# HKPolyU-UAV/MLMapping

Measured on NVIDIA B200. Metric: rays_integrated_per_sec, higher is better.
Workload: dtype f64

## Files before the change

### mlmapping_b200/csrc/explore_kernels.cuh

```cuda
#pragma once
#include "frame_kernels.cuh"
#include "order_kernels.cuh"

namespace mlm {

__device__ __forceinline__ bool inside_exp_bd(const MapParams &P, double x, double y, double z) {
  return x >= P.bd[0] && x < P.bd[1] && y >= P.bd[2] && y < P.bd[3] && z >= P.bd[4] && z < P.bd[5];
}

__device__ __forceinline__ void miss_tkey_body(const MapParams &P, DeviceBuffers &D, const FrameParams &F) {
  const FrameCounters *fc = D.fc[F.parity];
  const int n = fc->n_miss_list;
  const uint32_t *am = D.act_miss[F.parity];
  for (int j = blockIdx.x * blockDim.x + threadIdx.x; j < n; j += gridDim.x * blockDim.x) {
    const unsigned long long key = ((unsigned long long)am[D.miss_bucket[j]] << 32) | D.miss_t[j];
    atomicMax(&D.lvg_tkey[D.miss_lv[j]], key);
  }
}

__device__ __forceinline__ void nb_of(const MapParams &P, int dir, const int g[3], int sub, int gn[3], int &subn, int dl[3]) {
  int c[3] = {sub % P.n, (sub / P.n) % P.n, sub / (P.n * P.n)};
  gn[0] = g[0];
  gn[1] = g[1];
  gn[2] = g[2];
// ... 49 lines not shown
      if (!pack_glb(gn, hkey)) {
        fc->error = kErrRange;
        continue;
      }
      uint32_t slot = ht_hash(hkey) & P.ht_mask;
      int val = kBlockPending, created = -1;
      bool found = false;
      for (uint32_t probe = 0; probe <= P.ht_mask; probe++) {
        uint64_t k = D.ht_key[slot];
        if (k == kEmptyKey) {
          unsigned long long old = atomicCAS(reinterpret_cast<unsigned long long *>(&D.ht_key[slot]),
                                             (unsigned long long)kEmptyKey, (unsigned long long)hkey);
          if (old == kEmptyKey) {
            int top = atomicSub(D.free_top, 1) - 1;
            if (top < 0) {
              atomicAdd(D.free_top, 1);
              D.ht_val[slot] = kBlockUnusable;
              fc->error = kErrPool;
            } else {
              created = D.free_stack[top];
              D.ht_val[slot] = created;
              atomicAdd(&fc->n_new_blocks, 1);
            }
            val = kBlockPending;
            found = true;
            break;
          }
          k = (uint64_t)old;
        }
        if (k == hkey) {
          val = D.ht_val[slot];
          found = true;
          break;
        }
        slot = (slot + 1) & P.ht_mask;
      }
      if (!found) {
        fc->error = kErrPool;
        continue;
      }
      if (val == kBlockCollapsed || val == kBlockUnusable) continue;
      bool is_u = true;
      if (val >= 0) {
        is_u = D.pool_occ[(size_t)val * P.cell_stride + subn] == 'u';
        if (is_u) {
          const int cn[3] = {c[0] + dl[0], c[1] + dl[1], c[2] + dl[2]};
          const int lx = cn[0] - F.lvg_base[0], ly = cn[1] - F.lvg_base[1], lz = cn[2] - F.lvg_base[2];
          if ((unsigned)lx < (unsigned)P.lvg_dim_xy && (unsigned)ly < (unsigned)P.lvg_dim_xy && (unsigned)lz < (unsigned)P.lvg_dim_z) {
            const int lvn = (lz * P.lvg_dim_xy + ly) * P.lvg_dim_xy + lx;
            if (D.lvg[lvn].y > 0 && D.lvg_tkey[lvn] > my_key) is_u = false;
          }
        }
      }
      if (is_u) {
        const int blk = val >= 0 ? val : created;
        if (blk >= 0) atomicOr(&D.pool_front[(size_t)blk * P.front_words + (subn >> 5)], 1u << (subn & 31));
        else D.miss_choice[j] = (signed char)i;
        break;
      }
    }
  }
}

__device__ __forceinline__ void explore_b_body(const MapParams &P, DeviceBuffers &D, const FrameParams &F) {
  const FrameCounters *fc = D.fc[F.parity];
  const int n = fc->n_miss_list;
  const int dxy = P.lvg_dim_xy;
  for (int j = blockIdx.x * blockDim.x + threadIdx.x; j < n; j += gridDim.x * blockDim.x) {
    const int i = D.miss_choice[j];
    if (i < 0) continue;
    const int lv = D.miss_lv[j];
    int c[3] = {lv % dxy + F.lvg_base[0], (lv / dxy) % dxy + F.lvg_base[1], lv / (dxy * dxy) + F.lvg_base[2]};
    int g[3], l[3];
    for (int a = 0; a < 3; a++) {
      g[a] = floor_div(c[a], P.n);
      l[a] = c[a] - g[a] * P.n;
    }
    int gn[3], subn, dl[3];
    nb_of(P, i, g, (l[2] * P.n + l[1]) * P.n + l[0], gn, subn, dl);
    const int val = ht_find(P, D, gn);
    if (val >= 0) atomicOr(&D.pool_front[(size_t)val * P.front_words + (subn >> 5)], 1u << (subn & 31));
  }
}

__device__ __forceinline__ void release_body(const MapParams &P, DeviceBuffers &D, const FrameParams &F) {
  FrameCounters *fc = D.fc[F.parity];
  const int lane = lane_id();
  const int warp = (blockIdx.x * blockDim.x + threadIdx.x) >> 5, nwarps = (gridDim.x * blockDim.x) >> 5;
  const int n = fc->n_obs;
  for (int o = warp; o < n; o += nwarps) {
    const int ls = D.obs_list[o];
    if (lane == 0) D.obs_flag[ls] = 0;
    int lx = ls % P.lsg_dim_xy, ly = (ls / P.lsg_dim_xy) % P.lsg_dim_xy, lz = ls / (P.lsg_dim_xy * P.lsg_dim_xy);
    int g[3] = {lx + F.lsg_base[0], ly + F.lsg_base[1], lz + F.lsg_base[2]};
    uint32_t slot;
    const int block = ht_find_slot(P, D, g, slot);
    if (block < 0) continue;
    const size_t base = (size_t)block * P.cell_stride;
    bool ok = true;
    for (int w = lane; w < P.front_words; w += 32) ok &= D.pool_front[(size_t)block * P.front_words + w] == 0;
    const char first = D.pool_occ[base];
    if ((base & 3) == 0) {
      const uint32_t first4 = 0x01010101u * (uint32_t)(unsigned char)first;
      const uint32_t *occ4 = reinterpret_cast<const uint32_t *>(D.pool_occ + base);
      const int n4 = P.cells >> 2;
      for (int i = lane; i < n4; i += 32) ok &= occ4[i] == first4;
      for (int i = (n4 << 2) + lane; i < P.cells; i += 32) ok &= D.pool_occ[base + i] == first;
    } else {
      for (int i = lane; i < P.cells; i += 32) ok &= D.pool_occ[base + i] == first;
    }
    if (!__all_sync(0xffffffffu, ok)) continue;
    if (lane == 0) {
      D.col_occ[slot] = first;
      D.col_inf[slot] = D.pool_inf[base];
      D.col_lo[slot] = D.pool_lo[base];
      D.ht_val[slot] = kBlockCollapsed;
      atomicAdd(&fc->n_released, 1);
    }
    __syncwarp();
    for (int i = lane; i < P.cell_stride; i += 32) {
      D.pool_occ[base + i] = 'u';
      D.pool_inf[base + i] = 'u';
      D.pool_lo[base + i] = 0.f;
    }
    for (int w = lane; w < P.front_words; w += 32) D.pool_front[(size_t)block * P.front_words + w] = 0;
    __syncwarp();
    if (lane == 0) {
      __threadfence();
      D.free_stack[atomicAdd(D.free_top, 1)] = block;
    }
  }
}

__global__ void __launch_bounds__(256) k_miss_finalize(MapParams P, DeviceBuffers D, FrameParams F) { miss_finalize_body(P, D, F); }
__global__ void __launch_bounds__(256) k_miss_tkey(MapParams P, DeviceBuffers D, FrameParams F) { miss_tkey_body(P, D, F); }
__global__ void __launch_bounds__(256) k_explore_a(MapParams P, DeviceBuffers D, FrameParams F) { explore_a_body(P, D, F); }
__global__ void __launch_bounds__(256) k_explore_b(MapParams P, DeviceBuffers D, FrameParams F) { explore_b_body(P, D, F); }
__global__ void __launch_bounds__(256) k_release(MapParams P, DeviceBuffers D, FrameParams F) { release_body(P, D, F); }

template <int kMode>
__global__ void __launch_bounds__(kColThreads, 1) k_frame_explore(MapParams P, DeviceBuffers D, FrameParams F) {
  extern __shared__ __align__(16) unsigned char s_raw[];
  const int G = (int)gridDim.x;
  FrameCounters *fc = D.fc[F.parity];
  MLM_FRAME_WALL(0);
  {
    const int n_tiles = (F.n_total + F.tile_pts - 1) / F.tile_pts;
    for (int t = blockIdx.x; t < max(n_tiles, 1); t += G) {
      project_tile<kMode>(P, D, F, t, reinterpret_cast<int *>(s_raw));
      __syncthreads();
    }
  }
  MLM_FRAME_WALL(1);
  grid_barrier(D.grid_bar, G);
  MLM_FRAME_WALL(2);
  column_phase(P, D, F, s_raw);
  MLM_FRAME_WALL(3);
  grid_barrier(D.grid_bar, 2 * G);
  MLM_FRAME_WALL(4);
  if (blockIdx.x == 0 && threadIdx.x == 0) *D.col_queue = 0;
  miss_finalize_body(P, D, F);
  if (__ldcg(&fc->n_hit) > (int)F.bucket_count || __ldcg(&fc->n_miss_list) > (int)F.bucket_count_miss) {
    frame_bail(D, fc, F);
    return;
  }
  fuse_body<1>(P, D, F);
  MLM_FRAME_WALL(5);
  grid_barrier(D.grid_bar, 3 * G);
  miss_tkey_body(P, D, F);
  MLM_FRAME_WALL(6);
  grid_barrier(D.grid_bar, 4 * G);
  explore_a_body(P, D, F);
  MLM_FRAME_WALL(9);
  grid_barrier(D.grid_bar, 5 * G);
  explore_b_body(P, D, F);
  MLM_FRAME_WALL(10);
  fuse_body<2, false>(P, D, F);
  MLM_FRAME_WALL(11);
  grid_barrier(D.grid_bar, 6 * G);
  release_body(P, D, F);
  MLM_FRAME_WALL(12);
  frame_finish(P, D, F, fc, __ldcg(&fc->n_hit));
}

}
```

### mlmapping_b200/csrc/frame_kernels.cuh

```cuda
#pragma once
#include "exact_math.cuh"
#include "types.cuh"

namespace mlm {


__device__ __forceinline__ int cvt_trunc_x86(double x) {
  if (!(x > -2147483649.0 && x < 2147483648.0)) return (int)0x80000000;
  return __double2int_rz(x);
}

__device__ __forceinline__ int lane_id() { return threadIdx.x & 31; }

__device__ __forceinline__ int round_to_int_x86(double v) {
  if (!(v > -2147483000.0 && v < 2147483000.0)) return cvt_trunc_x86(round(v));
  int zi = __double2int_rz(v);
  double frac = v - (double)zi;
  if (frac >= 0.5) zi++;
  else if (frac <= -0.5) zi--;
  return zi;
}

__device__ __forceinline__ int agg_inc(int *ctr) {
  unsigned mask = __activemask();
// ... 547 lines not shown
    __syncwarp();
  }
  __syncthreads();
}

__device__ __forceinline__ void resolve_one(const MapParams &P, const FrameParams &F, DeviceBuffers &D, FrameCounters *fc,
                                            const int ls, const bool rearm_flag) {
  int block = -3;
  int lx = ls % P.lsg_dim_xy, ly = (ls / P.lsg_dim_xy) % P.lsg_dim_xy, lz = ls / (P.lsg_dim_xy * P.lsg_dim_xy);
  int g[3] = {lx + F.lsg_base[0], ly + F.lsg_base[1], lz + F.lsg_base[2]};
  uint64_t key;
  if (!pack_glb(g, key)) {
    fc->error = kErrRange;
  } else {
    uint32_t slot = ht_hash(key) & P.ht_mask;
    bool done = false;
    for (uint32_t probe = 0; probe <= P.ht_mask && !done; probe++) {
      uint64_t k = __ldcg(&D.ht_key[slot]);
      if (k == kEmptyKey) {
        unsigned long long old = atomicCAS(reinterpret_cast<unsigned long long *>(&D.ht_key[slot]),
                                           (unsigned long long)kEmptyKey, (unsigned long long)key);
        if (old == kEmptyKey) {
          int top = atomicSub(D.free_top, 1) - 1;
          if (top < 0) {
            atomicAdd(D.free_top, 1);
            D.ht_val[slot] = -3;
            fc->error = kErrPool;
          } else {
            block = D.free_stack[top];
            D.ht_val[slot] = block;
            atomicAdd(&fc->n_new_blocks, 1);
          }
          done = true;
          break;
        }
        k = (uint64_t)old;
      }
      if (k == key) {
        block = __ldcg(&D.ht_val[slot]);
        if (block == kBlockUnusable) fc->error = kErrPool;
        done = true;
        break;
      }
      slot = (slot + 1) & P.ht_mask;
    }
    if (!done) fc->error = kErrPool;
  }
  D.lsg_block[ls] = block;
  if (rearm_flag) D.lsg_flag[ls] = 0;
}
__device__ __forceinline__ void resolve_subboxes(const MapParams &P, const FrameParams &F, DeviceBuffers &D,
                                                 FrameCounters *fc, int first, int stride) {
  const int n = *reinterpret_cast<volatile int *>(&fc->n_touched_sub);
  for (int i = first; i < n; i += stride) resolve_one(P, F, D, fc, __ldcg(&D.touched_sub[i]), true);
}

__device__ __forceinline__ void touch_subbox(const MapParams &P, const FrameParams &F, DeviceBuffers &D,
                                             FrameCounters *fc, const int g[3]) {
  int ls = lsg_index(P, F, g);
  if (ls < 0) {
    fc->error = kErrInternal;
    return;
  }
  if (__ldcg(&D.lsg_flag[ls]) == 0) {
    if (atomicExch(&D.lsg_flag[ls], 1) == 0) {
      int pos = atomicAdd(&fc->n_touched_sub, 1);
      D.touched_sub[pos] = ls;
      if (F.inline_resolve) resolve_one(P, F, D, fc, ls, false);
    }
  }
}

struct WalkStart {
  double rate;
  int rho, z;
};
__device__ __forceinline__ WalkStart walk_prepare(const MapParams &P, int rho, int z) {
  WalkStart ws;
  ws.rate = (rho < P.nRho && z >= 0 && z < P.nZ) ? __ldg(&P.rate_table[z * P.nRho + rho]) : ray_rate(P, rho, z);
  if (rho >= P.nRho) {
    z = round_to_int_x86((double)z - (double)(rho - P.nRho + 1) * ws.rate);
    rho = P.nRho - 1;
  }
  ws.rho = rho;
  ws.z = z;
  return ws;
}
__device__ __forceinline__ void walk_mark(const MapParams &P, uint32_t *s_miss, double rate, int rho, int z,
                                          uint32_t *stamp_col, uint32_t t) {
  const int lane = lane_id();
  const double zd = (double)z;
  const int w_top = (rho - 1) >> 5;
  double diff = (double)(rho - (w_top << 5) - lane);
  for (int w = w_top; w >= 0; --w, diff += 32.0) {
    const int r = (w << 5) + lane;
    bool valid = r >= 1 && r <= rho - 1;
    const int zc = round_to_int_x86(zd - diff * rate);
    valid = valid && zc >= 0 && zc < P.nZ;
    if (stamp_col && valid) atomicMin(&stamp_col[zc * P.nRho + r], t * (uint32_t)P.nRho + (uint32_t)(rho - 1 - r));
    const int key = valid ? zc : -1;
    const int prev = __shfl_up_sync(0xffffffffu, key, 1);
    const unsigned heads = __ballot_sync(0xffffffffu, lane == 0 || key != prev);
    if (valid && (lane == 0 || key != prev)) {
      const unsigned rest = lane < 31 ? heads >> (lane + 1) : 0u;
      const int len = rest ? __ffs(rest) : 32 - lane;
      const unsigned mask = (len >= 32 ? 0xffffffffu : ((1u << len) - 1u)) << lane;
      uint32_t *wp = &s_miss[zc * P.words_per_row + w];
      if ((*reinterpret_cast<volatile uint32_t *>(wp) & mask) != mask) atomicOr(wp, mask);
    }
  }
}
__device__ __forceinline__ void walk_batch(const MapParams &P, uint32_t *s_miss, bool need, int rho, int z,
                                           uint32_t *stamp_col = nullptr, uint32_t t = 0) {
  WalkStart ws;
  ws.rate = 0.0;
  ws.rho = 0;
  ws.z = 0;
  if (need) ws = walk_prepare(P, rho, z);
  unsigned todo = __ballot_sync(0xffffffffu, need);
  while (todo) {
    const int src = __ffs(todo) - 1;
    todo &= todo - 1;
    const double rate = __shfl_sync(0xffffffffu, ws.rate, src);
    const int r0 = __shfl_sync(0xffffffffu, ws.rho, src);
    const int z0 = __shfl_sync(0xffffffffu, ws.z, src);
    const uint32_t t0 = __shfl_sync(0xffffffffu, t, src);
    walk_mark(P, s_miss, rate, r0, z0, stamp_col, t0);
  }
}

__device__ __forceinline__ void group_bar(int id, int count) { asm volatile("bar.sync %0, %1;" ::"r"(id), "r"(count) : "memory"); }

__device__ __forceinline__ void compact_bits(const uint32_t *bm, int w0, int w1, uint32_t *list, int *counter, int warp,
                                             int nwarps) {
  const int lane = lane_id();
  for (int wi = w0 + warp; wi < w1; wi += nwarps) {
    const uint32_t bits = bm[wi];
    if (!bits) continue;
    int base = 0;
    if (lane == 0) base = atomicAdd(counter, __popc(bits));
    base = __shfl_sync(0xffffffffu, base, 0);
    if ((bits >> lane) & 1u) list[base + __popc(bits & ((1u << lane) - 1))] = ((uint32_t)wi << 5) | (uint32_t)lane;
  }
}

__host__ __device__ inline size_t col_smem_prefix_bytes(int col_words, int nRho, int nCol) {
  return (((size_t)2 * col_words + kCntTotal + kColWarps + (size_t)kOddsRows * nRho + nRho + kMapCap) * 4 + (size_t)nCol * 2 + 15) & ~(size_t)15;
}

#ifdef MLM_PHASE_TIMING
#define MLM_PHASE(i) do { __syncthreads(); if (threadIdx.x == 0) D.debug_cycles[vc * 16 + (i)] = clock64(); } while (0)
#define MLM_PHASE_G(i, leader) do { if (threadIdx.x == (leader)) D.debug_cycles[vc * 16 + (i)] = clock64(); } while (0)
#define MLM_WALL(i) do { if (threadIdx.x == 0) { unsigned long long t_; asm volatile("mov.u64 %0, %%globaltimer;" : "=l"(t_)); D.debug_cycles[vc * 16 + (i)] = (long long)t_; } } while (0)
#else
#define MLM_WALL(i) do { } while (0)
#define MLM_PHASE(i) do { } while (0)
#define MLM_PHASE_G(i, leader) do { } while (0)
#endif

constexpr uint32_t kMissStampPending = 0xffffffffu;
__device__ __forceinline__ void miss_finalize_body(const MapParams &P, DeviceBuffers &D, const FrameParams &F) {
  if (!P.explore || !P.split) return;
  const FrameCounters *fc = D.fc[F.parity];
  const int n = __ldcg(&fc->n_miss_list);
  const int per_z = P.nRho * P.nPhi;
  for (int j = blockIdx.x * blockDim.x + threadIdx.x; j < n; j += gridDim.x * blockDim.x) {
    if (__ldcg(&D.miss_t[j]) != kMissStampPending) continue;
    const int idx = __ldcg(&D.miss_idx[j]);
    const int z = idx / per_z, rem = idx - z * per_z;
    const int phi = rem / P.nRho, r = rem - phi * P.nRho;
    const uint32_t st = __ldcg(&D.miss_stamp[((size_t)phi * P.nZ + z) * P.nRho + r]);
    D.miss_t[j] = st;
    atomicMin(&D.act_miss[F.parity][__ldcg(&D.miss_bucket[j])], st);
  }
}

__device__ __forceinline__ void column_item(const MapParams &P, DeviceBuffers &D, const FrameParams &F, const int item,
                                            unsigned char *s_raw) {
  FrameCounters *fc = D.fc[F.parity];
  uint32_t *act = D.act[F.parity];
  const bool merged = P.split && item >= P.nCol;
  const int phi = merged ? item - P.nCol : (P.split ? item >> 1 : item);
  const int side = (P.split && !merged) ? (item & 1) : -1;
  const int vc = merged ? 2 * phi : item;
  const int vc2 = merged ? vc + 1 : -1;
  const int z_own_lo = side == 1 ? P.n_below + 1 : 0;
  const int z_own_hi = side == 0 ? P.n_below : P.nZ;
  const int z_shared = side >= 0 ? P.n_below : -1;
  const int tid = threadIdx.x;
  const int n_c = D.phi_hist[vc] + (merged ? D.phi_hist[vc2] : 0);
  uint32_t *g_miss = D.miss_bitmap + (size_t)phi * P.col_words;
  MLM_PHASE(15);
  MLM_WALL(13);
  uint32_t *s_miss = reinterpret_cast<uint32_t *>(s_raw);
  uint32_t *s_end = s_miss + P.col_words;
  uint32_t *s_cnt = s_end + P.col_words;
  uint32_t *s_wsum = s_cnt + kCntTotal;
  float *s_odds = reinterpret_cast<float *>(s_wsum + kColWarps);
  int *s_reach = reinterpret_cast<int *>(s_odds + kOddsRows * P.nRho);
  int *s_map = s_reach + P.nRho;
  uint64_t *s_keys = reinterpret_cast<uint64_t *>(s_raw + col_smem_prefix_bytes(P.col_words, P.nRho, P.nCol));
  uint32_t *end_t_col = P.explore ? D.end_t + (size_t)phi * P.nZ * P.nRho : nullptr;
  uint32_t *stamp_col = P.explore ? D.miss_stamp + (size_t)phi * P.nZ * P.nRho : nullptr;
  if (P.explore) {
    const int e_lo = side == 1 ? P.n_below : z_own_lo;
    for (int i = e_lo * P.nRho + tid; i < z_own_hi * P.nRho; i += blockDim.x) end_t_col[i] = 0xffffffffu;
    for (int i = z_own_lo * P.nRho + tid; i < z_own_hi * P.nRho; i += blockDim.x)
      if (!P.split || i < P.n_below * P.nRho || i >= (P.n_below + 1) * P.nRho) stamp_col[i] = 0xffffffffu;
  }
  __shared__ int s_warp[33];
  __shared__ int s_off;
  const int bound_c = D.phi_bound[vc] + (merged ? D.phi_bound[vc2] : 0);
  const bool in_smem = bound_c <= P.sort_cap_smem;
  const bool big = n_c > P.map_cap;
  int off = 0;
  if (big || !in_smem) {
    int part = 0;
    for (int p = tid; p < vc; p += blockDim.x) part += D.phi_hist[p];
    for (int ofs = 16; ofs > 0; ofs >>= 1) part += __shfl_xor_sync(0xffffffffu, part, ofs);
    if (tid == 0) s_off = 0;
    __syncthreads();
    if (lane_id() == 0 && part) atomicAdd(&s_off, part);
    __syncthreads();
    off = s_off;
  }
  {
    const int nb = (F.n_total + F.tile_pts - 1) / F.tile_pts;
    const int per = (nb + (int)blockDim.x - 1) / (int)blockDim.x;
    const int b0 = min(tid * per, nb), b1 = min(b0 + per, nb);
    uint32_t dsave[4], dsave2[4];
    int mine = 0;
#pragma unroll
    for (int q = 0; q < 4; q++) {
      dsave[q] = 0;
      dsave2[q] = 0;
      if (b0 + q < b1) {
        dsave[q] = __ldcg(&D.rec_dir[(size_t)(b0 + q) * P.nCol + vc]);
        mine += (int)(dsave[q] & 0xffffu);
        if (merged) {
          dsave2[q] = __ldcg(&D.rec_dir[(size_t)(b0 + q) * P.nCol + vc2]);
          mine += (int)(dsave2[q] & 0xffffu);
        }
      }
    }
    for (int b = b0 + 4; b < b1; b++) {
      mine += (int)(__ldcg(&D.rec_dir[(size_t)b * P.nCol + vc]) & 0xffffu);
      if (merged) mine += (int)(__ldcg(&D.rec_dir[(size_t)b * P.nCol + vc2]) & 0xffffu);
    }
    int incl = mine;
    const int lane = lane_id(), w = tid >> 5, nw = blockDim.x >> 5;
#pragma unroll
    for (int ofs = 1; ofs < 32; ofs <<= 1) {
      int t = __shfl_up_sync(0xffffffffu, incl, ofs);
      if (lane >= ofs) incl += t;
    }
    if (lane == 31) s_warp[w] = incl;
    __syncthreads();
    if (w == 0) {
      int sv = lane < nw ? s_warp[lane] : 0, si = sv;
#pragma unroll
      for (int ofs = 1; ofs < 32; ofs <<= 1) {
        int t = __shfl_up_sync(0xffffffffu, si, ofs);
        if (lane >= ofs) si += t;
      }
      if (lane < nw) s_warp[lane] = si - sv;
    }
    __syncthreads();
    int dst = s_warp[w] + incl - mine;
    for (int b = b0; b < b1; b++) {
      for (int half = 0; half < (merged ? 2 : 1); half++) {
        const int col = half ? vc2 : vc;
        const uint32_t d = b - b0 < 4 ? (half ? dsave2[b - b0] : dsave[b - b0]) : __ldcg(&D.rec_dir[(size_t)b * P.nCol + col]);
        const int c = (int)(d & 0xffffu);
        const int src = b * F.tile_pts + (int)(d >> 16);
        for (int r = 0; r < c; r++) {
          if (big) D.rec_col[off + dst + r] = D.rec_lin[src + r];
          else s_map[dst + r] = src + r;
        }
        dst += c;
      }
    }
  }
  __syncthreads();
  const RayRecord *recs = big ? D.rec_col + off : D.rec_lin;
#define REC_AT(i) recs[big ? (i) : s_map[i]]
  MLM_PHASE(0);

  __shared__ int s_nk;
  __shared__ int s_nmiss;
  __shared__ int s_nhead;
  __shared__ int s_nlist;
  for (int i = tid; i < 2 * P.col_words; i += blockDim.x) s_miss[i] = 0;
  if (tid == 0) {
    s_nk = 0;
    s_nmiss = 0;
    s_nhead = 0;
  }
  __syncthreads();
  uint64_t *keys = in_smem ? s_keys : D.col_scratch + (size_t)2 * off * P.contrib_per_point;
  uint64_t *keys_alt = in_smem ? s_keys + P.sort_cap_smem : keys + (size_t)n_c * P.contrib_per_point;
  int kbits = 1;
  while ((1 << kbits) < n_c) kbits++;
  const int cell_shift = 12 + kbits;
  const int cell_sentinel = 1 << P.cell_bits;
  __syncthreads();

  MLM_PHASE(1);
// ... 162 lines not shown
    const int hcap = 4096;
    uint32_t *s_list = s_cnt + hcap;
    const int list_cap = kCntTotal - hcap;
    const int words_per_chunk = max(1, list_cap >> 5);
    const int gt = tid - nFold;

    if (P.visibility_check) {
      const int warp = gt >> 5, nwarps = nWalk >> 5;
      for (int w0 = 0; w0 < P.col_words; w0 += words_per_chunk) {
        if (gt == 0) s_nlist = 0;
        group_bar(2, nWalk);
        compact_bits(s_end, w0, min(w0 + words_per_chunk, P.col_words), s_list, &s_nlist, warp, nwarps);
        group_bar(2, nWalk);
        const int n_list = s_nlist;
        for (int it = 0; it * 32 * nwarps < n_list; it++) {
          const int k = (it * 32 + lane_id()) * nwarps + warp;
          int rho = 0, z = 0;
          if (k < n_list) {
            const uint32_t e = s_list[k];
            const int wi = (int)(e >> 5), wr = wi - (wi / P.words_per_row) * P.words_per_row;
            z = wi / P.words_per_row;
            rho = (wr << 5) + (int)(e & 31);
          }
          walk_batch(P, s_miss, k < n_list, rho, z, stamp_col,
                     (P.explore && k < n_list) ? end_t_col[z * P.nRho + rho] : 0u);
        }
        group_bar(2, nWalk);
      }
      for (int i = gt; i < hcap; i += nWalk) s_hash[i] = 0xffffffffu;
      group_bar(2, nWalk);
      MLM_PHASE_G(9, nFold);
      for (int it = 0; it * 32 * nwarps < n_c; it++) {
        const int i = (it * 32 + lane_id()) * nwarps + warp;
        RayRecord rc;
        rc.phi_flags = kRecInside;
        if (i < n_c) rc = REC_AT(i);
        bool need = !(rc.phi_flags & kRecInside);
        if (need && !P.explore && rc.rho < 65536 && rc.z >= -32768 && rc.z < 32768) {
          const uint32_t key = ((uint32_t)rc.rho << 16) | (uint32_t)(rc.z + 32768);
          uint32_t slot = (key * 2654435761u) >> 7;
          for (int probe = 0; probe < 8; probe++) {
            slot &= (uint32_t)(hcap - 1);
            uint32_t old = atomicCAS(&s_hash[slot], 0xffffffffu, key);
            if (old == 0xffffffffu) break;
            if (old == key) {
              need = false;
              break;
            }
            slot++;
          }
        }
        walk_batch(P, s_miss, need, rc.rho, rc.z, stamp_col, rc.t);
      }
      group_bar(2, nWalk);
      MLM_PHASE_G(12, nFold);
    }
  }
#ifdef MLM_PHASE_TIMING
#endif
  __syncthreads();

  MLM_PHASE(6);
  uint32_t *s_list = reinterpret_cast<uint32_t *>(s_keys);
  uint32_t *s_tout = s_list + P.sort_cap_smem * 2;
  __shared__ int s_tcnt, s_tbase, s_rcnt, s_rbase, s_mbase;
  const int list_cap = P.sort_cap_smem * 2;
  const int words_per_chunk = max(1, list_cap >> 5);
  for (int wi = z_own_lo * P.words_per_row + tid; wi < z_own_hi * P.words_per_row; wi += blockDim.x) g_miss[wi] = s_miss[wi];
  if (z_shared >= 0) {
    if (tid < P.words_per_row) {
      const int wi = z_shared * P.words_per_row + tid;
      const uint32_t mine = s_miss[wi];
      if (mine) s_miss[wi] = mine & ~atomicOr(&g_miss[wi], mine);
    }
    __syncthreads();
  }
  const int stage_w0 = min(z_own_lo, z_shared >= 0 ? z_shared : z_own_lo) * P.words_per_row;
  const int stage_w1 = max(z_own_hi, z_shared + 1) * P.words_per_row;
  for (int w0 = stage_w0; w0 < stage_w1; w0 += words_per_chunk) {
    if (tid == 0) {
      s_nk = 0;
      s_tcnt = 0;
      s_rcnt = 0;
    }
    __syncthreads();
    compact_bits(s_miss, w0, min(w0 + words_per_chunk, stage_w1), s_list, &s_nk, tid >> 5, (int)blockDim.x >> 5);
    __syncthreads();
    const int n_list = s_nk;
    if (P.explore) {
      if (tid == 0) s_mbase = n_list ? atomicAdd(&fc->n_miss_list, n_list) : 0;
      __syncthreads();
    }
    for (int k = tid; k < n_list; k += blockDim.x) {
      const uint32_t e = s_list[k];
      const int wi = (int)(e >> 5), z = wi / P.words_per_row, wr = wi - z * P.words_per_row;
      const int r = (wr << 5) + (int)(e & 31);
      double2 cxy = __ldg(&P.centre_xy[phi * P.nRho + r]);
      CellRef cr = locate_cell(P, cxy.x + F.t_wa[0], cxy.y + F.t_wa[1], __ldg(&P.centre_z[z]) + F.t_wa[2]);
      int lv = lvg_index(P, F, cr);
      if (P.explore) {
        const int idx_cell = (z * P.nPhi + phi) * P.nRho + r;
        const bool pending = P.split && z == P.n_below;
        const uint32_t st = pending ? kMissStampPending : stamp_col[z * P.nRho + r];
        const uint32_t bkt = (uint32_t)idx_cell % F.bucket_count_miss;
        if (!pending) atomicMin(&D.act_miss[F.parity][bkt], st);
        const int j = s_mbase + k;
        D.miss_idx[j] = idx_cell;
        D.miss_lv[j] = lv < 0 ? 0 : lv;
        D.miss_t[j] = st;
        D.miss_bucket[j] = bkt;
      }
      if (lv < 0) {
        fc->error = kErrInternal;
        continue;
      }
      int old = atomicAdd(&D.lvg[lv].y, 1);
      const bool remote = F.stage_only && subbox_owner(cr.g, F.shard_world) != F.shard_rank;
      if (old == 0) {
        if (!remote) s_tout[agg_inc(&s_tcnt)] = (uint32_t)lv;
        else s_tout[list_cap - 1 - agg_inc(&s_rcnt)] = (uint32_t)lv;
      }
      if (!remote) touch_subbox(P, F, D, fc, cr.g);
    }
    __syncthreads();
    const int n_t = s_tcnt, n_r = s_rcnt;
    if (tid == 0) {
      s_nmiss += n_list;
      if (n_t) s_tbase = atomicAdd(&fc->n_touched, n_t);
    }
    if (tid == 32 && n_r) s_rbase = atomicAdd(&fc->n_touched_remote, n_r);
    __syncthreads();
    if (n_t) {
      const int tb = s_tbase;
      if (tb + n_t > P.max_touched) fc->error = kErrCapacity;
      for (int i = tid; i < n_t && tb + i < P.max_touched; i += blockDim.x) D.touched[tb + i] = s_tout[i];
    }
    if (n_r) {
      const int rb = s_rbase;
      if (rb + n_r > P.max_touched) fc->error = kErrCapacity;
      for (int i = tid; i < n_r && rb + i < P.max_touched; i += blockDim.x) D.touched_remote[rb + i] = s_tout[list_cap - 1 - i];
    }
    __syncthreads();
  }
  MLM_PHASE(7);
  MLM_WALL(14);
#ifdef MLM_PHASE_TIMING
  if (tid == 0) { D.debug_cycles[vc * 16 + 10] = n_c; D.debug_cycles[vc * 16 + 11] = n_k; }
#endif
  if (tid == 0 && s_nmiss) atomicAdd(&fc->n_miss, s_nmiss);
}

__device__ __forceinline__ int column_weight(const DeviceBuffers &D, int vc) { return 4 * D.phi_hist[vc] + D.phi_bound[vc]; }

__device__ __forceinline__ void column_phase(const MapParams &P, DeviceBuffers &D, const FrameParams &F, unsigned char *s_raw) {
  const int tid = threadIdx.x;
  __shared__ int s_item, s_wmax, s_nactive;
  uint32_t *s_cnt = reinterpret_cast<uint32_t *>(s_raw) + 2 * P.col_words;
  uint32_t *s_wsum = s_cnt + kCntTotal;
  float *s_odds = reinterpret_cast<float *>(s_wsum + kColWarps);
  int *s_reach = reinterpret_cast<int *>(s_odds + kOddsRows * P.nRho);
  uint16_t *s_order = reinterpret_cast<uint16_t *>(s_reach + P.nRho + kMapCap);
  uint64_t *s_keys = reinterpret_cast<uint64_t *>(s_raw + col_smem_prefix_bytes(P.col_words, P.nRho, P.nCol));
  for (int i = tid; i < kOddsRows * P.nRho; i += blockDim.x) s_odds[i] = __ldg(&P.odds_table[i]);
  for (int i = tid; i < P.nRho; i += blockDim.x) s_reach[i] = __ldg(&P.k_reach[i]);
  if (tid == 0) {
    s_wmax = 0;
    s_nactive = 0;
  }
  __syncthreads();
  int *s_nrec = reinterpret_cast<int *>(s_keys);
  int *s_wgt = s_nrec + P.nCol;
  const bool sorted = P.nCol <= P.sort_cap_smem;
  auto not_mine = [&](int vc) {
    const int phi = P.split ? vc >> 1 : vc;
    return F.shard_world > 1 && (phi % F.shard_world) != F.shard_rank;
  };
  if (sorted) {
    int my_active = 0;
    for (int vc = tid; vc < P.nCol; vc += blockDim.x) {
      const int n = not_mine(vc) ? 0 : D.phi_hist[vc];
      const int w = n > 0 ? column_weight(D, vc) : 0;
      s_nrec[vc] = n;
      s_wgt[vc] = w;
      if (n > 0) {
        my_active++;
        atomicMax(&s_wmax, w);
      }
    }
    if (my_active) atomicAdd(&s_nactive, my_active);
  }
  __syncthreads();
  constexpr int kCovered = (int)0x80000000;
  if (sorted && P.split && P.merge && s_nactive > (int)gridDim.x) {
    __shared__ int s_mh[64];
    __shared__ int s_T, s_sh2, s_need;
    if (tid < 64) s_mh[tid] = 0;
    if (tid == 0) {
      int sh2 = 0;
      while (((2 * s_wmax) >> sh2) > 63) sh2++;
      s_sh2 = sh2;
    }
    __syncthreads();
    const int sh2 = s_sh2;
    for (int phi = tid; phi < P.nPhi; phi += blockDim.x)
      if (s_nrec[2 * phi] > 0 && s_nrec[2 * phi + 1] > 0) atomicAdd(&s_mh[(s_wgt[2 * phi] + s_wgt[2 * phi + 1]) >> sh2], 1);
    __syncthreads();
    if (tid == 0) {
      int c2 = 0;
      for (int b = 0; b < 64; b++) c2 += s_mh[b];
      const int need = min(c2, s_nactive - (int)gridDim.x);
      int cum = 0, T = -1;
      for (int b = 0; b < 64 && need > 0; b++) {
        cum += s_mh[b];
        if (cum >= need) {
          T = b;
          break;
        }
      }
      s_T = T;
      s_need = need;
    }
    __syncthreads();
    const int need = s_need;
    int *s_rank = reinterpret_cast<int *>(s_keys + P.sort_cap_smem);
    int below = 0;
    for (int b = 0; b < s_T; b++) below += s_mh[b];
    const int take = need - below;
    for (int phi = tid; phi < P.nPhi; phi += blockDim.x) {
      const int n0 = s_nrec[2 * phi], n1 = s_nrec[2 * phi + 1];
      s_rank[phi] = (n0 > 0 && n1 > 0 && ((s_wgt[2 * phi] + s_wgt[2 * phi + 1]) >> sh2) == s_T) ? 1 : 0;
    }
    __syncthreads();
    __shared__ int s_scan_warp[33];
    block_exclusive_scan(s_rank, P.nPhi, s_scan_warp);
    int merged_here = 0;
    for (int phi = tid; phi < P.nPhi; phi += blockDim.x) {
      const int n0 = s_nrec[2 * phi], n1 = s_nrec[2 * phi + 1];
      if (n0 > 0 && n1 > 0) {
        const int w = s_wgt[2 * phi] + s_wgt[2 * phi + 1];
        const int bkt = w >> sh2;
        if (bkt < s_T || (bkt == s_T && s_rank[phi] < take)) {
          s_wgt[2 * phi] = w;
          s_nrec[2 * phi] = -(n0 + n1);
          s_nrec[2 * phi + 1] = kCovered;
          merged_here++;
          atomicMax(&s_wmax, w);
        }
      }
    }
    if (merged_here) atomicSub(&s_nactive, merged_here);
    __syncthreads();
  }
  auto is_active = [&](int vc) { return sorted ? s_nrec[vc] != 0 : (D.phi_hist[vc] > 0 && !not_mine(vc)); };
  for (int vc = blockIdx.x; vc < P.nCol; vc += gridDim.x) {
    if (is_active(vc)) continue;
    const int phi = P.split ? vc >> 1 : vc, side = P.split ? (vc & 1) : -1;
    const int z_lo = side == 1 ? P.n_below + 1 : 0, z_hi = side == 0 ? P.n_below : P.nZ;
    uint32_t *g_miss = D.miss_bitmap + (size_t)phi * P.col_words;
    for (int i = z_lo * P.words_per_row + tid; i < z_hi * P.words_per_row; i += blockDim.x) g_miss[i] = 0;
  }
  int n_active = 0;
  if (sorted) {
    n_active = s_nactive;
    int sh = 0;
    while ((s_wmax >> sh) > 63) sh++;
    uint64_t *q_src = s_keys + P.sort_cap_smem;
    uint64_t kq[8];
    int nk = 0;
    for (int vc = tid; vc < P.nCol && nk < 8; vc += blockDim.x) {
      const int nr = s_nrec[vc];
      const bool item = nr != 0 && nr != kCovered;
      kq[nk++] = ((item ? (uint64_t)(63 - (s_wgt[vc] >> sh)) : 64ull) << 16) | (uint64_t)(nr < 0 ? P.nCol + (vc >> 1) : vc);
    }
    __syncthreads();
    nk = 0;
    for (int vc = tid; vc < P.nCol && nk < 8; vc += blockDim.x) q_src[vc] = kq[nk++];
    __syncthreads();
    radix_pass(q_src, s_keys, P.nCol, 16, 7, s_cnt, s_wsum);
    for (int i = tid; i < n_active; i += blockDim.x) s_order[i] = (uint16_t)(s_keys[i] & 0xffffu);
  } else {
    n_active = P.nCol;
  }
#ifdef MLM_PHASE_TIMING
  if (threadIdx.x == 0) { unsigned long long t_; asm volatile("mov.u64 %0, %%globaltimer;" : "=l"(t_)); D.debug_cycles[(P.nCol + blockIdx.x) * 16 + 7] = (long long)t_; }
#endif
  bool first_round = true;
  for (;;) {
    __syncthreads();
    if (tid == 0) s_item = first_round ? (int)blockIdx.x : atomicAdd(D.col_queue, 1) + (int)gridDim.x;
    first_round = false;
    __syncthreads();
    const int item = s_item;
    if (item >= n_active) break;
    const int vc = sorted ? (int)s_order[item] : item;
    if (!sorted && !is_active(vc)) continue;
    column_item(P, D, F, vc, s_raw);
  }
}

__global__ void __launch_bounds__(kColThreads, 1) k_column(MapParams P, DeviceBuffers D, FrameParams F) {
  extern __shared__ __align__(16) unsigned char s_raw[];
  FrameCounters *fc = D.fc[F.parity];
  const int tid = threadIdx.x;
  __shared__ int s_last;
  column_phase(P, D, F, s_raw);
  __threadfence();
  __syncthreads();
  if (tid == 0) s_last = atomicAdd(D.col_ticket, 1) == (int)gridDim.x - 1;
  __syncthreads();
  if (s_last) {
    if (tid == 0) {
      *D.col_ticket = 0;
      *D.col_queue = 0;
    }
    __threadfence();
    if (!F.stage_only) resolve_subboxes(P, F, D, fc, threadIdx.x, blockDim.x);
  }
}

constexpr int kBucketChainLen = 24;
__device__ __constant__ uint32_t c_bucket_chain[kBucketChainLen] = {
    1,      13,     29,      59,      127,     257,      541,      1109,     2357,     5087,     10273,   20753,
    42043,  85229,  172933,  351061,  712697,  1447153,  2938679,  5967347,  12117689, 24607243, 49969847, 101473717};

__device__ __forceinline__ void publish_counters(const DeviceBuffers &D, FrameCounters *fc, uint32_t frame_seq = 0) {
  const int lane = threadIdx.x & 31;
  const int n = (int)(sizeof(FrameCounters) / sizeof(int)) - 1;
  for (int i = lane; i < n; i += 32) reinterpret_cast<volatile int *>(D.host_fc)[i] = __ldcg(reinterpret_cast<const int *>(fc) + i);
  __syncwarp();
  if (lane == 0 && frame_seq) {
    __threadfence_system();
    *reinterpret_cast<volatile uint32_t *>(&D.host_fc->seq) = frame_seq;
  }
}

constexpr int kFuseLocal = 16;
__device__ __forceinline__ void frame_bail(const DeviceBuffers &D, FrameCounters *fc, const FrameParams &F) {
  __shared__ int s_ovf_last;
  if (threadIdx.x == 0) {
    s_ovf_last = atomicAdd(D.fuse_ticket, 1) == (int)gridDim.x - 1;
    if (s_ovf_last) {
      *D.fuse_ticket = 0;
      *D.grid_bar = 0;
      fc->overflow = 1;
      __threadfence();
    }
  }
  __syncthreads();
  if (s_ovf_last && threadIdx.x < 32) publish_counters(D, fc, F.frame_seq);
}

__device__ __forceinline__ void frame_finish(const MapParams &P, DeviceBuffers &D, const FrameParams &F, FrameCounters *fc, int n_hit_frame);

template <int kPhase, bool kFinish = true>
__device__ __forceinline__ void fuse_body(const MapParams &P, DeviceBuffers &D, const FrameParams &F) {
  if (F.skip_flag && __ldcg(F.skip_flag)) return;
  FrameCounters *fc = D.fc[F.parity];
  const uint32_t *act = D.act[F.parity];
  const int n_hit_frame = fc->n_hit;
  if (kPhase == 0 && F.order_mode == 0 && n_hit_frame > (int)F.bucket_count) {
    frame_bail(D, fc, F);
    return;
  }
  const int n = min(fc->n_touched, P.max_touched);
  const int dxy = P.lvg_dim_xy;
  const unsigned long long kClaimed64 = (unsigned long long)(uint32_t)kLvgClaimed;
  const unsigned long long kEmpty64 = (unsigned long long)(uint32_t)kLvgEmpty;
  int my_touched = 0, my_obs = 0;
  const int fw_ = (int)(threadIdx.x >> 5), fl_ = (int)(threadIdx.x & 31);
  for (int i = ((fw_ * (int)gridDim.x + (int)blockIdx.x) << 5) + fl_; i < n; i += (int)gridDim.x * (int)blockDim.x) {
    const uint32_t e = D.touched[i];
    if (e == 0xffffffffu) continue;
    const int lv = (int)(e & ~kTouchedHitTag);
    int c[3], g[3], sub;
    {
      const int lz = (int)fast_div((uint32_t)lv, P.dxy2_mul, P.dxy2_shift);
      const int rem = lv - lz * dxy * dxy;
      const int ly = (int)fast_div((uint32_t)rem, P.dxy_mul, P.dxy_shift);
      c[0] = rem - ly * dxy + F.lvg_base[0];
      c[1] = ly + F.lvg_base[1];
      c[2] = lz + F.lvg_base[2];
      int l[3];
      for (int a = 0; a < 3; a++) {
        g[a] = fast_floor_div(c[a], P.n, P.n_mul, P.n_shift);
        l[a] = c[a] - g[a] * P.n;
      }
      sub = (l[2] * P.n + l[1]) * P.n + l[0];
    }
    const int ls = lsg_index(P, F, g);
    const int block = ls >= 0 ? __ldcg(&D.lsg_block[ls]) : -3;
    unsigned long long *slot = reinterpret_cast<unsigned long long *>(&D.lvg[lv]);
    int head, mc;
    bool counted_by_hits = false;
    if (kPhase == 1) {
      if (!(e & kTouchedHitTag)) continue;
      head = D.lvg[lv].x;
      mc = 0;
    } else {
      const unsigned long long old = atomicExch(slot, kClaimed64);
      head = (int)(uint32_t)old;
      mc = (int)(old >> 32);
      if (head == kLvgClaimed) {
        *slot = kEmpty64;
        continue;
      }
      if (!(head != kLvgEmpty && mc > 0)) *slot = kEmpty64;
      if (kPhase == 2) {
        counted_by_hits = head != kLvgEmpty;
        head = kLvgEmpty;
        D.lvg_tkey[lv] = 0ull;
      }
    }
    if (block < 0) continue;
    const size_t addr = (size_t)block * P.cell_stride + sub;
    float lo = D.pool_lo[addr];
    char occ = D.pool_occ[addr];
    if (!counted_by_hits) my_touched++;
    bool became_o = false, became_f = false;

    if (head != kLvgEmpty) {
      uint64_t st0 = 0, st1 = 0, st2 = 0, st3 = 0;
      float p0 = 0.f, p1 = 0.f, p2 = 0.f, p3 = 0.f;
      int cnt = 0;
      uint64_t ls[kFuseLocal];
      float lp[kFuseLocal];
      for (int h = head; h != kLvgEmpty; h = D.hit_next[h]) {
        if (cnt < kFuseLocal) {
          const uint64_t st = ((uint64_t)act[D.hit_bucket[h]] << 32) | D.hit_t[h];
          const float ph = D.hit_p[h];
          if (cnt == 0) { st0 = st; p0 = ph; }
          else if (cnt == 1) { st1 = st; p1 = ph; }
          else if (cnt == 2) { st2 = st; p2 = ph; }
          else if (cnt == 3) { st3 = st; p3 = ph; }
          else { ls[cnt] = st; lp[cnt] = ph; }
        }
        cnt++;
      }
      auto apply_hit = [&](float ph) {
        if (lo < P.lo_max) {
          lo = __fadd_rn(lo, logit_f(ph, P.log10f_fma));
          lo = lo > P.lo_max ? P.lo_max : lo;
        }
        if (lo > P.lo_sh && occ != 'o') {
          occ = 'o';
          my_obs++;
          became_o = true;
        }
      };
      if (cnt <= 4) {
#define MLM_CSWAP(sa, pa, sb, pb) if (sa < sb) { uint64_t ts = sa; sa = sb; sb = ts; float tp = pa; pa = pb; pb = tp; }
        MLM_CSWAP(st0, p0, st1, p1) MLM_CSWAP(st2, p2, st3, p3) MLM_CSWAP(st0, p0, st2, p2)
        MLM_CSWAP(st1, p1, st3, p3) MLM_CSWAP(st1, p1, st2, p2)
#undef MLM_CSWAP
        apply_hit(p0);
        if (cnt > 1) apply_hit(p1);
        if (cnt > 2) apply_hit(p2);
        if (cnt > 3) apply_hit(p3);
      } else if (cnt <= kFuseLocal) {
        ls[0] = st0; lp[0] = p0;
        ls[1] = st1; lp[1] = p1;
        ls[2] = st2; lp[2] = p2;
        ls[3] = st3; lp[3] = p3;
        for (int m = 1; m < cnt; m++) {
          const uint64_t st = ls[m];
          const float ph = lp[m];
          int j = m;
          while (j > 0 && ls[j - 1] < st) {
            ls[j] = ls[j - 1];
            lp[j] = lp[j - 1];
            j--;
          }
          ls[j] = st;
          lp[j] = ph;
        }
        for (int k = 0; k < cnt; k++) apply_hit(lp[k]);
      } else {
        uint64_t prev = ~0ull;
        for (int k = 0; k < cnt; k++) {
          uint64_t best = 0;
          int hb = -1;
          for (int q = head; q != kLvgEmpty; q = D.hit_next[q]) {
            const uint64_t st = ((uint64_t)act[D.hit_bucket[q]] << 32) | D.hit_t[q];
            if (st < prev && (hb < 0 || st > best)) {
              best = st;
              hb = q;
            }
          }
          prev = best;
          apply_hit(D.hit_p[hb]);
        }
      }
    }
    for (int k = 0; k < mc; k++) {
      bool changed = false;
      if (lo >= P.lo_min) {
        float nl = __fadd_rn(lo, P.lo_miss);
        nl = nl < P.lo_min ? P.lo_min : nl;
        changed = nl != lo;
        lo = nl;
      }
      if (lo < P.lo_sh && occ != 'f') {
        occ = 'f';
        changed = true;
        became_f = true;
      }
      if (!changed) break;
    }
    D.pool_lo[addr] = lo;
    D.pool_occ[addr] = occ;
    if (P.explore && (became_o || became_f))
      atomicAnd(&D.pool_front[(size_t)block * P.front_words + (sub >> 5)], ~(1u << (sub & 31)));
  }
  __shared__ int s_ctr[2];
  if (threadIdx.x < 2) s_ctr[threadIdx.x] = 0;
  __syncthreads();
  for (int ofs = 16; ofs > 0; ofs >>= 1) {
    my_touched += __shfl_xor_sync(0xffffffffu, my_touched, ofs);
    my_obs += __shfl_xor_sync(0xffffffffu, my_obs, ofs);
  }
  if (lane_id() == 0) {
    if (my_touched) atomicAdd(&s_ctr[0], my_touched);
    if (my_obs) atomicAdd(&s_ctr[1], my_obs);
  }
  __syncthreads();
  if (threadIdx.x == 0) {
    if (s_ctr[0]) atomicAdd(&fc->n_touched_voxels, s_ctr[0]);
    if (s_ctr[1]) atomicAdd(&fc->obs_delta, s_ctr[1]);
  }
  if (kPhase == 1 || !kFinish) return;
  frame_finish(P, D, F, fc, n_hit_frame);
}

__device__ __forceinline__ void frame_finish(const MapParams &P, DeviceBuffers &D, const FrameParams &F, FrameCounters *fc, int n_hit_frame) {
  if (blockIdx.x == 0 && threadIdx.x == 0) fc->fused = 1;
  {
    __shared__ int s_is_last;
    __threadfence();
    __syncthreads();
#ifdef MLM_PHASE_TIMING
    if (threadIdx.x == 0) { unsigned long long t_; asm volatile("mov.u64 %0, %%globaltimer;" : "=l"(t_)); D.debug_cycles[(P.nCol + blockIdx.x) * 16 + 8] = (long long)t_; }
#endif
    if (threadIdx.x == 0) s_is_last = atomicAdd(D.fuse_ticket, 1) == (int)gridDim.x - 1;
    __syncthreads();
    if (s_is_last && threadIdx.x < 32) {
      if (threadIdx.x == 0) {
        *D.fuse_ticket = 0;
        *D.grid_bar = 0;
        fc->fused = 1;
        __threadfence();
      }
      __syncwarp();
      publish_counters(D, fc, F.frame_seq);
    }
  }

  {
    const int gtid = blockIdx.x * blockDim.x + threadIdx.x, nth = gridDim.x * blockDim.x;
    uint32_t B = F.bucket_count;
    const uint32_t n_hit = (uint32_t)n_hit_frame;
    if (n_hit > 0 && B == 1) B = 13;
    for (int c = 0; c + 1 < kBucketChainLen && n_hit > B; c++)
      if (c_bucket_chain[c] == B) B = c_bucket_chain[c + 1];
    uint32_t *act_next = D.act[F.parity ^ 1];
    for (uint32_t i = gtid; i < B; i += nth) act_next[i] = 0xffffffffu;
    if (P.explore) {
      uint32_t Bm = F.bucket_count_miss;
      const uint32_t n_miss = (uint32_t)fc->n_miss_list;
      if (n_miss > 0 && Bm == 1) Bm = 13;
      for (int c = 0; c + 1 < kBucketChainLen && n_miss > Bm; c++)
        if (c_bucket_chain[c] == Bm) Bm = c_bucket_chain[c + 1];
      uint32_t *am = D.act_miss[F.parity ^ 1];
      for (uint32_t i = gtid; i < Bm; i += nth) am[i] = 0xffffffffu;
    }
    if (F.inline_resolve) {
      const int nts = fc->n_touched_sub;
      for (int i = gtid; i < nts; i += nth) D.lsg_flag[__ldcg(&D.touched_sub[i])] = 0;
    }
    for (int i = gtid; i < P.nCol; i += nth) {
      D.phi_hist[i] = 0;
      D.phi_bound[i] = 0;
    }
    if (P.explore && P.split)
      for (int i = gtid; i < P.nPhi * P.nRho; i += nth) {
        const int phi = i / P.nRho, r = i - phi * P.nRho;
        D.miss_stamp[((size_t)phi * P.nZ + P.n_below) * P.nRho + r] = 0xffffffffu;
      }
    if (gtid < (int)(sizeof(FrameCounters) / sizeof(int))) reinterpret_cast<int *>(D.fc[F.parity ^ 1])[gtid] = 0;
  }
}

template <int kPhase>
__global__ void __launch_bounds__(256) k_fuse(MapParams P, DeviceBuffers D, FrameParams F) {
  fuse_body<kPhase>(P, D, F);
}

__device__ __forceinline__ void grid_barrier(int *counter, int target) {
  __syncthreads();
  if (threadIdx.x == 0) {
    __threadfence();
    atomicAdd(counter, 1);
    int v;
    do {
      asm volatile("ld.acquire.gpu.global.s32 %0, [%1];" : "=r"(v) : "l"(counter) : "memory");
    } while (v < target);
    __threadfence();
  }
  __syncthreads();
}

#ifdef MLM_PHASE_TIMING
#define MLM_FRAME_WALL(i) do { if (threadIdx.x == 0) { unsigned long long t_; asm volatile("mov.u64 %0, %%globaltimer;" : "=l"(t_)); D.debug_cycles[(P.nCol + blockIdx.x) * 16 + (i)] = (long long)t_; } } while (0)
#else
#define MLM_FRAME_WALL(i) do { } while (0)
#endif
template <int kMode>
__global__ void __launch_bounds__(kColThreads, 1) k_frame(MapParams P, DeviceBuffers D, FrameParams F) {
  extern __shared__ __align__(16) unsigned char s_raw[];
  const int G = (int)gridDim.x;
  MLM_FRAME_WALL(0);
  {
    const int n_tiles = (F.n_total + F.tile_pts - 1) / F.tile_pts;
    for (int t = blockIdx.x; t < max(n_tiles, 1); t += G) {
      project_tile<kMode>(P, D, F, t, reinterpret_cast<int *>(s_raw));
      __syncthreads();
    }
  }
  MLM_FRAME_WALL(1);
  grid_barrier(D.grid_bar, G);
  MLM_FRAME_WALL(2);
  column_phase(P, D, F, s_raw);
  MLM_FRAME_WALL(3);
  grid_barrier(D.grid_bar, 2 * G);
  MLM_FRAME_WALL(4);
  MLM_FRAME_WALL(5);
  if (blockIdx.x == 0 && threadIdx.x == 0) *D.col_queue = 0;
  fuse_body<0>(P, D, F);
  MLM_FRAME_WALL(6);
}

}
```

Baseline: 3.510 billion.

## Split grid barrier to overlap table loads; replace radix sort with rank sort

Splits the grid barrier into arrive and wait, so each block loads the odds and reach tables into shared memory while waiting for the other blocks. The merge-threshold selection now uses a warp-level scan and ballot instead of a serial loop by thread 0, plus an inline ballot-based rank in place of a block exclusive scan. Column ordering drops the 64-bit radix pass and instead packs active columns into 32-bit keys and sorts them with a quadratic brute-force rank count. The rank sort adds O(n_active^2) shared-memory reads, which could become costly when many columns are active.

```diff
diff --git a/mlmapping_b200/csrc/explore_kernels.cuh b/mlmapping_b200/csrc/explore_kernels.cuh
--- a/mlmapping_b200/csrc/explore_kernels.cuh
+++ b/mlmapping_b200/csrc/explore_kernels.cuh
@@ -225,9 +225,11 @@
     }
   }
   MLM_FRAME_WALL(1);
-  grid_barrier(D.grid_bar, G);
+  grid_arrive(D.grid_bar);
+  load_col_tables(P, s_raw);
+  grid_wait(D.grid_bar, G);
   MLM_FRAME_WALL(2);
-  column_phase(P, D, F, s_raw);
+  column_phase(P, D, F, s_raw, true);
   MLM_FRAME_WALL(3);
   grid_barrier(D.grid_bar, 2 * G);
   MLM_FRAME_WALL(4);
diff --git a/mlmapping_b200/csrc/frame_kernels.cuh b/mlmapping_b200/csrc/frame_kernels.cuh
--- a/mlmapping_b200/csrc/frame_kernels.cuh
+++ b/mlmapping_b200/csrc/frame_kernels.cuh
@@ -723,7 +723,9 @@
 #define MLM_PHASE(i) do { __syncthreads(); if (threadIdx.x == 0) D.debug_cycles[vc * 16 + (i)] = clock64(); } while (0)
 #define MLM_PHASE_G(i, leader) do { if (threadIdx.x == (leader)) D.debug_cycles[vc * 16 + (i)] = clock64(); } while (0)
 #define MLM_WALL(i) do { if (threadIdx.x == 0) { unsigned long long t_; asm volatile("mov.u64 %0, %%globaltimer;" : "=l"(t_)); D.debug_cycles[vc * 16 + (i)] = (long long)t_; } } while (0)
+#define MLM_FRAME_WALL(i) do { if (threadIdx.x == 0) { unsigned long long t_; asm volatile("mov.u64 %0, %%globaltimer;" : "=l"(t_)); D.debug_cycles[(P.nCol + blockIdx.x) * 16 + (i)] = (long long)t_; } } while (0)
 #else
+#define MLM_FRAME_WALL(i) do { } while (0)
 #define MLM_WALL(i) do { } while (0)
 #define MLM_PHASE(i) do { } while (0)
 #define MLM_PHASE_G(i, leader) do { } while (0)
@@ -1192,22 +1194,30 @@
 
 __device__ __forceinline__ int column_weight(const DeviceBuffers &D, int vc) { return 4 * D.phi_hist[vc] + D.phi_bound[vc]; }
 
-__device__ __forceinline__ void column_phase(const MapParams &P, DeviceBuffers &D, const FrameParams &F, unsigned char *s_raw) {
-  const int tid = threadIdx.x;
-  __shared__ int s_item, s_wmax, s_nactive;
-  uint32_t *s_cnt = reinterpret_cast<uint32_t *>(s_raw) + 2 * P.col_words;
-  uint32_t *s_wsum = s_cnt + kCntTotal;
-  float *s_odds = reinterpret_cast<float *>(s_wsum + kColWarps);
+__device__ __forceinline__ void load_col_tables(const MapParams &P, unsigned char *s_raw) {
+  float *s_odds = reinterpret_cast<float *>(s_raw) + 2 * P.col_words + kCntTotal + kColWarps;
   int *s_reach = reinterpret_cast<int *>(s_odds + kOddsRows * P.nRho);
-  uint16_t *s_order = reinterpret_cast<uint16_t *>(s_reach + P.nRho + kMapCap);
+  for (int i = threadIdx.x; i < kOddsRows * P.nRho; i += blockDim.x) s_odds[i] = __ldg(&P.odds_table[i]);
+  for (int i = threadIdx.x; i < P.nRho; i += blockDim.x) s_reach[i] = __ldg(&P.k_reach[i]);
+}
+
+__device__ __forceinline__ void column_phase(const MapParams &P, DeviceBuffers &D, const FrameParams &F, unsigned char *s_raw,
+                                             bool tables_loaded = false) {
+  const int tid = threadIdx.x, lane = tid & 31, warp = tid >> 5;
+  __shared__ int s_item, s_wmax, s_nactive, s_nq;
+  __shared__ int s_mh[64];
+  uint16_t *s_order = reinterpret_cast<uint16_t *>(reinterpret_cast<int *>(s_raw) + 2 * P.col_words + kCntTotal + kColWarps +
+                                                   kOddsRows * P.nRho + P.nRho + kMapCap);
   uint64_t *s_keys = reinterpret_cast<uint64_t *>(s_raw + col_smem_prefix_bytes(P.col_words, P.nRho, P.nCol));
-  for (int i = tid; i < kOddsRows * P.nRho; i += blockDim.x) s_odds[i] = __ldg(&P.odds_table[i]);
-  for (int i = tid; i < P.nRho; i += blockDim.x) s_reach[i] = __ldg(&P.k_reach[i]);
+  if (!tables_loaded) load_col_tables(P, s_raw);
+  if (tid < 64) s_mh[tid] = 0;
   if (tid == 0) {
     s_wmax = 0;
     s_nactive = 0;
-  }
-  __syncthreads();
+    s_nq = 0;
+  }
+  __syncthreads();
+  MLM_FRAME_WALL(13);
   int *s_nrec = reinterpret_cast<int *>(s_keys);
   int *s_wgt = s_nrec + P.nCol;
   const bool sorted = P.nCol <= P.sort_cap_smem;
@@ -1230,67 +1240,70 @@
     if (my_active) atomicAdd(&s_nactive, my_active);
   }
   __syncthreads();
+  MLM_FRAME_WALL(14);
   constexpr int kCovered = (int)0x80000000;
   if (sorted && P.split && P.merge && s_nactive > (int)gridDim.x) {
-    __shared__ int s_mh[64];
-    __shared__ int s_T, s_sh2, s_need;
-    if (tid < 64) s_mh[tid] = 0;
-    if (tid == 0) {
-      int sh2 = 0;
-      while (((2 * s_wmax) >> sh2) > 63) sh2++;
-      s_sh2 = sh2;
-    }
-    __syncthreads();
-    const int sh2 = s_sh2;
+    __shared__ int s_T, s_need, s_below;
+    __shared__ int s_wc[32];
+    int sh2 = 0;
+    while (((2 * s_wmax) >> sh2) > 63) sh2++;
     for (int phi = tid; phi < P.nPhi; phi += blockDim.x)
       if (s_nrec[2 * phi] > 0 && s_nrec[2 * phi + 1] > 0) atomicAdd(&s_mh[(s_wgt[2 * phi] + s_wgt[2 * phi + 1]) >> sh2], 1);
     __syncthreads();
-    if (tid == 0) {
-      int c2 = 0;
-      for (int b = 0; b < 64; b++) c2 += s_mh[b];
+    if (warp == 0) {
+      const int m0 = s_mh[2 * lane], m1 = s_mh[2 * lane + 1];
+      int cum = m0 + m1;
+#pragma unroll
+      for (int ofs = 1; ofs < 32; ofs <<= 1) {
+        const int t = __shfl_up_sync(0xffffffffu, cum, ofs);
+        if (lane >= ofs) cum += t;
+      }
+      const int c2 = __shfl_sync(0xffffffffu, cum, 31);
       const int need = min(c2, s_nactive - (int)gridDim.x);
-      int cum = 0, T = -1;
-      for (int b = 0; b < 64 && need > 0; b++) {
-        cum += s_mh[b];
-        if (cum >= need) {
-          T = b;
-          break;
-        }
-      }
-      s_T = T;
-      s_need = need;
+      const int cum0 = cum - m1;
+      const unsigned hit = __ballot_sync(0xffffffffu, need > 0 && cum >= need);
+      const int L = hit ? __ffs(hit) - 1 : 0;
+      const int cum0_L = __shfl_sync(0xffffffffu, cum0, L), m0_L = __shfl_sync(0xffffffffu, m0, L);
+      if (lane == 0) {
+        const bool first = cum0_L >= need;
+        s_T = hit ? (first ? 2 * L : 2 * L + 1) : -1;
+        s_below = hit ? (first ? cum0_L - m0_L : cum0_L) : 0;
+        s_need = need;
+      }
     }
     __syncthreads();
-    const int need = s_need;
-    int *s_rank = reinterpret_cast<int *>(s_keys + P.sort_cap_smem);
-    int below = 0;
-    for (int b = 0; b < s_T; b++) below += s_mh[b];
-    const int take = need - below;
-    for (int phi = tid; phi < P.nPhi; phi += blockDim.x) {
-      const int n0 = s_nrec[2 * phi], n1 = s_nrec[2 * phi + 1];
-      s_rank[phi] = (n0 > 0 && n1 > 0 && ((s_wgt[2 * phi] + s_wgt[2 * phi + 1]) >> sh2) == s_T) ? 1 : 0;
-    }
-    __syncthreads();
-    __shared__ int s_scan_warp[33];
-    block_exclusive_scan(s_rank, P.nPhi, s_scan_warp);
-    int merged_here = 0;
-    for (int phi = tid; phi < P.nPhi; phi += blockDim.x) {
-      const int n0 = s_nrec[2 * phi], n1 = s_nrec[2 * phi + 1];
-      if (n0 > 0 && n1 > 0) {
-        const int w = s_wgt[2 * phi] + s_wgt[2 * phi + 1];
-        const int bkt = w >> sh2;
-        if (bkt < s_T || (bkt == s_T && s_rank[phi] < take)) {
-          s_wgt[2 * phi] = w;
-          s_nrec[2 * phi] = -(n0 + n1);
-          s_nrec[2 * phi + 1] = kCovered;
-          merged_here++;
-          atomicMax(&s_wmax, w);
-        }
-      }
+    const int T = s_T;
+    const int take = s_need - s_below;
+    int merged_here = 0, run = 0;
+    for (int base = 0; base < P.nPhi; base += blockDim.x) {
+      const int phi = base + tid;
+      const bool both = phi < P.nPhi && s_nrec[2 * phi] > 0 && s_nrec[2 * phi + 1] > 0;
+      const int w = both ? s_wgt[2 * phi] + s_wgt[2 * phi + 1] : 0;
+      const int bkt = w >> sh2;
+      const unsigned at_t = __ballot_sync(0xffffffffu, both && bkt == T);
+      if (lane == 0) s_wc[warp] = __popc(at_t);
+      __syncthreads();
+      int wsum = lane < (int)(blockDim.x >> 5) ? s_wc[lane] : 0;
+#pragma unroll
+      for (int ofs = 1; ofs < 32; ofs <<= 1) {
+        const int t = __shfl_up_sync(0xffffffffu, wsum, ofs);
+        if (lane >= ofs) wsum += t;
+      }
+      const int rank = run + (warp ? __shfl_sync(0xffffffffu, wsum, warp - 1) : 0) + __popc(at_t & ((1u << lane) - 1));
+      run += __shfl_sync(0xffffffffu, wsum, 31);
+      if (both && (bkt < T || (bkt == T && rank < take))) {
+        s_wgt[2 * phi] = w;
+        s_nrec[2 * phi] = -(s_nrec[2 * phi] + s_nrec[2 * phi + 1]);
+        s_nrec[2 * phi + 1] = kCovered;
+        merged_here++;
+        atomicMax(&s_wmax, w);
+      }
+      __syncthreads();
     }
     if (merged_here) atomicSub(&s_nactive, merged_here);
     __syncthreads();
   }
+  MLM_FRAME_WALL(15);
   auto is_active = [&](int vc) { return sorted ? s_nrec[vc] != 0 : (D.phi_hist[vc] > 0 && !not_mine(vc)); };
   for (int vc = blockIdx.x; vc < P.nCol; vc += gridDim.x) {
     if (is_active(vc)) continue;
@@ -1304,26 +1317,29 @@
     n_active = s_nactive;
     int sh = 0;
     while ((s_wmax >> sh) > 63) sh++;
-    uint64_t *q_src = s_keys + P.sort_cap_smem;
-    uint64_t kq[8];
-    int nk = 0;
-    for (int vc = tid; vc < P.nCol && nk < 8; vc += blockDim.x) {
+    uint32_t *q_key = reinterpret_cast<uint32_t *>(s_keys + P.sort_cap_smem);
+    for (int vc = tid; vc < P.nCol; vc += blockDim.x) {
       const int nr = s_nrec[vc];
-      const bool item = nr != 0 && nr != kCovered;
-      kq[nk++] = ((item ? (uint64_t)(63 - (s_wgt[vc] >> sh)) : 64ull) << 16) | (uint64_t)(nr < 0 ? P.nCol + (vc >> 1) : vc);
-    }
+      if (nr != 0 && nr != kCovered)
+        q_key[agg_inc(&s_nq)] = ((uint32_t)(63 - (s_wgt[vc] >> sh)) << 24) | ((uint32_t)vc << 1) | (nr < 0 ? 1u : 0u);
+    }
+    if (tid < 3) q_key[n_active + tid] = 0xffffffffu;
     __syncthreads();
-    nk = 0;
-    for (int vc = tid; vc < P.nCol && nk < 8; vc += blockDim.x) q_src[vc] = kq[nk++];
-    __syncthreads();
-    radix_pass(q_src, s_keys, P.nCol, 16, 7, s_cnt, s_wsum);
-    for (int i = tid; i < n_active; i += blockDim.x) s_order[i] = (uint16_t)(s_keys[i] & 0xffffu);
+    const uint4 *q4 = reinterpret_cast<const uint4 *>(q_key);
+    for (int i = tid; i < n_active; i += blockDim.x) {
+      const uint32_t k = q_key[i];
+      int rank = 0;
+      for (int j = 0; j < (n_active + 3) >> 2; j++) {
+        const uint4 q = q4[j];
+        rank += (q.x < k) + (q.y < k) + (q.z < k) + (q.w < k);
+      }
+      const int vc = (int)((k >> 1) & 0x7fffffu);
+      s_order[rank] = (uint16_t)((k & 1u) ? P.nCol + (vc >> 1) : vc);
+    }
   } else {
     n_active = P.nCol;
   }
-#ifdef MLM_PHASE_TIMING
-  if (threadIdx.x == 0) { unsigned long long t_; asm volatile("mov.u64 %0, %%globaltimer;" : "=l"(t_)); D.debug_cycles[(P.nCol + blockIdx.x) * 16 + 7] = (long long)t_; }
-#endif
+  MLM_FRAME_WALL(7);
   bool first_round = true;
   for (;;) {
     __syncthreads();
@@ -1577,9 +1593,7 @@
     __shared__ int s_is_last;
     __threadfence();
     __syncthreads();
-#ifdef MLM_PHASE_TIMING
-    if (threadIdx.x == 0) { unsigned long long t_; asm volatile("mov.u64 %0, %%globaltimer;" : "=l"(t_)); D.debug_cycles[(P.nCol + blockIdx.x) * 16 + 8] = (long long)t_; }
-#endif
+    MLM_FRAME_WALL(8);
     if (threadIdx.x == 0) s_is_last = atomicAdd(D.fuse_ticket, 1) == (int)gridDim.x - 1;
     __syncthreads();
     if (s_is_last && threadIdx.x < 32) {
@@ -1634,11 +1648,15 @@
   fuse_body<kPhase>(P, D, F);
 }
 
-__device__ __forceinline__ void grid_barrier(int *counter, int target) {
+__device__ __forceinline__ void grid_arrive(int *counter) {
   __syncthreads();
   if (threadIdx.x == 0) {
     __threadfence();
     atomicAdd(counter, 1);
+  }
+}
+__device__ __forceinline__ void grid_wait(int *counter, int target) {
+  if (threadIdx.x == 0) {
     int v;
     do {
       asm volatile("ld.acquire.gpu.global.s32 %0, [%1];" : "=r"(v) : "l"(counter) : "memory");
@@ -1647,12 +1665,11 @@
   }
   __syncthreads();
 }
-
-#ifdef MLM_PHASE_TIMING
-#define MLM_FRAME_WALL(i) do { if (threadIdx.x == 0) { unsigned long long t_; asm volatile("mov.u64 %0, %%globaltimer;" : "=l"(t_)); D.debug_cycles[(P.nCol + blockIdx.x) * 16 + (i)] = (long long)t_; } } while (0)
-#else
-#define MLM_FRAME_WALL(i) do { } while (0)
-#endif
+__device__ __forceinline__ void grid_barrier(int *counter, int target) {
+  grid_arrive(counter);
+  grid_wait(counter, target);
+}
+
 template <int kMode>
 __global__ void __launch_bounds__(kColThreads, 1) k_frame(MapParams P, DeviceBuffers D, FrameParams F) {
   extern __shared__ __align__(16) unsigned char s_raw[];
@@ -1666,9 +1683,11 @@
     }
   }
   MLM_FRAME_WALL(1);
-  grid_barrier(D.grid_bar, G);
+  grid_arrive(D.grid_bar);
+  load_col_tables(P, s_raw);
+  grid_wait(D.grid_bar, G);
   MLM_FRAME_WALL(2);
-  column_phase(P, D, F, s_raw);
+  column_phase(P, D, F, s_raw, true);
   MLM_FRAME_WALL(3);
   grid_barrier(D.grid_bar, 2 * G);
   MLM_FRAME_WALL(4);
```

Result: faster. 3.697 billion, median of 6 (+5.3%).
